# ruanjinchen/Point-Cloud-Flow-Matching

Hardware: AMD Instinct MI355X
Metric: train-step points/sec (B=8, N=20000, xyz+rgb) at 1/2/4/8 MI355X; Chamfer ms (higher is better)
Workload: dtype fp32 ContextNet (scatter/gather ops fp32; Conv3d + 1x1 convs as bf16x3 split-operand matrix-core products, fp32 accumulate, ~2^-16 per product vs the reference's default cuDNN TF32 2^-11) + bf16 autocast per-point MLP head (reference AMP config; its per-cloud B-row layers -- embeddings, FiLM affines

## Files before the change

### point-cloud-flow-matching_amd/csrc/rows.hpp

```cpp
#pragma once

#include <algorithm>

#include "bn_chan.hpp"
#include "pcfm_common.hpp"

namespace pcfm {


struct ProvIdx1 {
  static constexpr int TAPS = 1;
  const int* idx;
  int ni;
  int nrows;
  __device__ __forceinline__ void get(int b, int i, bool, int (&id)[1], float (&wt)[1]) const {
    const int v = idx[(size_t)b * ni + i];
    const bool ok = (unsigned)v < (unsigned)nrows;
    id[0] = ok ? v : 0;
    wt[0] = ok ? 1.0f : 0.0f;
  }
};

struct ProvDevox {
  static constexpr int TAPS = 8;
// ... 291 lines not shown
    int id[T];
    float w[T];
    prov.get(b, i, primary, id, w);
    const float4 a = tap_sum4<T>(lds4, id, w);
    const float r[4] = {a.x, a.y, a.z, a.w};
#pragma unroll
    for (int k = 0; k < 4; ++k) {
      float acc = r[k];
      if (epi.scale != nullptr) acc *= sc[k];
      if (ab != nullptr) acc += abn ? fa[k].z(ad[k]) : ad[k];
      ob[(size_t)k * NI + i] = acc;
    }
  }
}


struct RowPlan {
  int threads = 512;
  int cpb = 1;
  int groups = 1;
  int psplit = 1;
  bool use_lds = true;
  size_t lds_bytes = 0;
};

constexpr int kLdsFloatsSmall = 16 * 1024;
constexpr int kLdsFloatsBig = 32 * 1024;

constexpr long long kGatherTargetBlocks = 2 * kCUs;
constexpr int kGather1Ipt = 2;
// ... 17 lines not shown
  p.groups = groups(p.cpb);
  const long long blocks = (long long)p.groups * B;
  if (blocks < target) {
    const int want = ceil_div(target, blocks);
    const int cap = std::max(1, ceil_div(NI, p.threads));
    p.psplit = std::min(want, cap);
  }
  p.lds_bytes = p.use_lds ? (size_t)p.cpb * V * sizeof(float) : 0;
  return p;
}

template <class Prov>
inline bool prov_has_side_outputs(const Prov&) { return false; }
inline bool prov_has_side_outputs(const ProvDevox& p) { return p.inds_out != nullptr; }

template <class Prov>
inline int launch_gather(const float* rows, float* out, int B, int C, int V, int NI, Prov prov,
                         hipStream_t st, const char* what, GatherEpi epi = GatherEpi{},
                         BnParam bn = BnParam{}) {
  if (B == 0 || NI == 0) return PCFM_OK;
  if (V == 0 && C > 0 && epi.add == nullptr) {
    hipError_t e = hipMemsetAsync(out, 0, (size_t)B * C * NI * sizeof(float), st);
    if (e != hipSuccess) {
      set_error("%s: hipMemsetAsync: %s", what, hipGetErrorString(e));
      return (int)e;
    }
    if (!prov_has_side_outputs(prov)) return PCFM_OK;
  }
  RowPlan p = plan_gather(B, C, V, NI);
  dim3 grid(p.psplit, p.groups, B);
  if (p.use_lds && p.cpb == 4 && C % 4 == 0 && p.threads == 512) {
    int e = allow_big_lds((const void*)gather_rows4_kernel<Prov>);
    if (e) return e;
    hipLaunchKernelGGL((gather_rows4_kernel<Prov>), grid, dim3(512), p.lds_bytes, st, rows, out, C,
                       V, NI, prov, epi, bn);
  } else if (p.use_lds && p.cpb == 1 && p.threads == 1024) {
    int e = allow_big_lds((const void*)gather_rows1_kernel<Prov, kGather1Ipt>);
    if (e) return e;
    hipLaunchKernelGGL((gather_rows1_kernel<Prov, kGather1Ipt>), grid, dim3(1024), p.lds_bytes, st,
                       rows, out, C, V, NI, prov, epi, bn);
  } else if (p.use_lds) {
    int e = allow_big_lds((const void*)gather_rows_kernel<Prov, true>);
// ... 16 lines not shown
```

### point-cloud-flow-matching_amd/csrc/voxel.hip

```cpp
#include "rows.hpp"
#include "segsum.hpp"

namespace pcfm {
namespace {

__global__ void __launch_bounds__(256)
    vox_ind_kernel(const int* __restrict__ coords, int n, int r, int* __restrict__ ind) {
  const int b = blockIdx.y;
  const int i = blockIdx.x * blockDim.x + threadIdx.x;
  if (i >= n) return;
  const int* cb = coords + (size_t)b * 3 * n;
  ind[(size_t)b * n + i] = cb[i] * r * r + cb[i + n] * r + cb[i + 2 * n];
}

bool cube_fits(int r, int* s) {
  if (r < 1) return false;
  const long long c = (long long)r * r * r;
  if (c > (1LL << 30)) return false;
  *s = (int)c;
  return true;
}

__global__ void __launch_bounds__(256)
    rows_dot_kernel(const float* __restrict__ a, const float* __restrict__ b, int len, float scale,
// ... 334 lines not shown
extern "C" int pcfm_trilinear_devoxelize_bwd_planned(const float* grad_y, const void* plan, int b,
                                                     int c, int n, int r, float* grad_x, void* ws,
                                                     size_t ws_bytes, void* stream) {
  int s = 0;
  PCFM_CHECK_ARG(b >= 0 && c >= 0 && n >= 0, "trilinear_devoxelize_bwd_planned: negative size");
  PCFM_CHECK_ARG(cube_fits(r, &s), "trilinear_devoxelize_bwd_planned: bad resolution %d", r);
  PCFM_CHECK_ARG(plan != nullptr && ws_bytes >= seg_apply_bytes(b, c, n, s, 8),
                 "trilinear_devoxelize_bwd_planned: workspace too small");
  if (b == 0) return PCFM_OK;
  const int e = seg_apply(8, grad_y, seg_plan_carve(const_cast<void*>(plan), b, n, s, 8), false,
                          r, b, c, n, s, grad_x, seg_apply_carve(ws, b, c, n, s, 8),
                          (hipStream_t)stream);
  return e ? e : check_launch("trilinear_devoxelize_bwd_planned");
}

__device__ __forceinline__ float se_group_sum(float v) {
#pragma unroll
  for (int o = 8; o > 0; o >>= 1) v += __shfl_xor(v, o, 64);
  return v;
}

__global__ void __launch_bounds__(1024)
    se_mlp_fwd_kernel(const float* __restrict__ m, const float* __restrict__ w1,
                      const float* __restrict__ w2, int b, int c, int h, float* __restrict__ hid,
                      float* __restrict__ s) {
  extern __shared__ float sh[];
  float* ms = sh;
  float* w1s = ms + b * c;
  float* w2t = w1s + h * c;
  float* hs = w2t + h * c;
// ... 132 lines not shown
```

### point-cloud-flow-matching_amd/modules/functional/voxelization.py

```python
from torch.autograd import Function

from modules.functional import backend as _be



def _voxelize(feats, vox, r):
    if feats.is_cuda:
        from pcfm import ops, plans
        if plans.ENABLED:
            plan = plans.voxel_plan(vox, r)
            return ops.avg_voxelize_forward_planned(feats, plan), plan.ind, plan.cnt
    return _be._backend.avg_voxelize_forward(feats, vox, r)

__all__ = ["avg_voxelize", "avg_voxelize_tee"]


class AvgVoxelization(Function):

    @staticmethod
    def forward(ctx, features, coords, resolution):
        feats = features.contiguous()
        vox = coords.int().contiguous()
        b, c = feats.shape[0], feats.shape[1]
        r = int(resolution)
        grid, ind, cnt = _voxelize(feats, vox, r)
# ... 7 lines not shown
        flat = grad_output.contiguous().view(b, c, -1)
        return _be._backend.avg_voxelize_backward(flat, ind, cnt), None, None


avg_voxelize = AvgVoxelization.apply


class AvgVoxelizationTee(Function):

    @staticmethod
    def forward(ctx, features, coords, resolution):
        feats = features.contiguous()
        vox = coords.int().contiguous()
        b, c = feats.shape[0], feats.shape[1]
        r = int(resolution)
        grid, ind, cnt = _voxelize(feats, vox, r)
        ctx.save_for_backward(ind, cnt)
        return grid.view(b, c, r, r, r), features.view_as(features)

    @staticmethod
    def backward(ctx, grad_grid, grad_feat):
        from pcfm import ops
        ind, cnt = ctx.saved_tensors
        b, c = grad_grid.shape[0], grad_grid.shape[1]
        flat = grad_grid.contiguous().view(b, c, -1)
        if grad_feat is None:
            return _be._backend.avg_voxelize_backward(flat, ind, cnt), None, None
        return ops.avg_voxelize_backward_add(flat, ind, cnt, grad_feat), None, None


avg_voxelize_tee = AvgVoxelizationTee.apply
```

### point-cloud-flow-matching_amd/pcfm/_lib.py

```python
from __future__ import annotations

import ctypes
import os
import threading

_HERE = os.path.dirname(os.path.abspath(__file__))
LIB_PATH = os.path.join(os.path.dirname(_HERE), "csrc", "libpcfm_hip.so")
LIB_PATH = os.environ.get("PCFM_LIB", LIB_PATH)

_P = ctypes.c_void_p
_I = ctypes.c_int
_F = ctypes.c_float
_Z = ctypes.c_size_t
_L = ctypes.c_longlong
_D = ctypes.c_double
_DP = ctypes.POINTER(ctypes.c_double)

SIGNATURES = {
    "pcfm_abi_version": (_I, []),
    "pcfm_last_error": (ctypes.c_char_p, []),
    "pcfm_avg_voxelize_fwd_workspace_bytes": (_Z, [_I, _I, _I, _I]),
    "pcfm_avg_voxelize_fwd": (_I, [_P, _P, _I, _I, _I, _I, _P, _P, _P, _P, _Z, _P]),
    "pcfm_avg_voxelize_bwd": (_I, [_P, _P, _P, _I, _I, _I, _I, _P, _P]),
    "pcfm_trilinear_devoxelize_fwd": (_I, [_P, _P, _I, _I, _I, _I, _I, _P, _P, _P, _P]),
# ... 157 lines not shown
}

OCCUPANCY_ABI_VERSION = 1

EMD_ND_SIGNATURES = {
    "pcfm_emd_nd_abi_version": (_I, []),
    "pcfm_emd_nd_supported": (_I, [_I]),
    "pcfm_emd_nd_workspace_bytes": (_Z, [_I, _I, _I, _I]),
    "pcfm_emd_nd_approxmatch_cost_f32": (_I, [_P, _P, _I, _I, _I, _I, _P, _P, _P, _Z, _P]),
    "pcfm_emd_nd_matchcost_f32": (_I, [_P, _P, _P, _I, _I, _I, _I, _P, _P, _Z, _P]),
    "pcfm_emd_nd_matchcost_bwd_f32": (_I, [_P, _P, _P, _P, _I, _I, _I, _I, _P, _P, _P, _Z, _P]),
}

EMD_ND_ABI_VERSION = 1

_lock = threading.Lock()
_lib = None


class PcfmError(RuntimeError):
    """A pcfm_* entry point returned a non-zero status."""


def load() -> ctypes.CDLL:
    global _lib
    if _lib is not None:
        return _lib
    with _lock:
        if _lib is None:
            if not os.path.exists(LIB_PATH):
                raise RuntimeError(
                    f"pcfm: HIP library {LIB_PATH} is not built; run "
                    "`python -c 'import __graft_entry__ as g; g.build()'` "
                    "(HIP tensors have no fallback)")
            lib = ctypes.CDLL(LIB_PATH)
            for table in (SIGNATURES, ND_SIGNATURES, CROSS_SIGNATURES, FPS_SIGNATURES,
                          OCCUPANCY_SIGNATURES, EMD_ND_SIGNATURES):
                for name, (res, args) in table.items():
                    fn = getattr(lib, name)
                    fn.restype = res
                    fn.argtypes = args
            v = lib.pcfm_abi_version()
            if v != ABI_VERSION:
                raise RuntimeError(f"pcfm: ABI version {v} != expected {ABI_VERSION}; rebuild")
            v = lib.pcfm_chamfer_nd_abi_version()
            if v != ND_ABI_VERSION:
                raise RuntimeError(f"pcfm: chamfer_nd ABI version {v} != expected "
                                   f"{ND_ABI_VERSION}; rebuild")
            v = lib.pcfm_chamfer_cross_abi_version()
            if v != CROSS_ABI_VERSION:
                raise RuntimeError(f"pcfm: chamfer_cross ABI version {v} != expected "
                                   f"{CROSS_ABI_VERSION}; rebuild")
            v = lib.pcfm_fps_abi_version()
            if v != FPS_ABI_VERSION:
                raise RuntimeError(f"pcfm: fps ABI version {v} != expected "
                                   f"{FPS_ABI_VERSION}; rebuild")
            v = lib.pcfm_occupancy_abi_version()
            if v != OCCUPANCY_ABI_VERSION:
                raise RuntimeError(f"pcfm: occupancy ABI version {v} != expected "
                                   f"{OCCUPANCY_ABI_VERSION}; rebuild")
            v = lib.pcfm_emd_nd_abi_version()
            if v != EMD_ND_ABI_VERSION:
                raise RuntimeError(f"pcfm: emd_nd ABI version {v} != expected "
                                   f"{EMD_ND_ABI_VERSION}; rebuild")
            _lib = lib
    return _lib


def call(name: str, *args) -> None:
    lib = load()
    rc = getattr(lib, name)(*args)
    if rc != 0:
        msg = lib.pcfm_last_error().decode(errors="replace")
        raise PcfmError(f"{name} failed (status {rc}): {msg}")


def query(name: str, *args) -> int:
    return int(getattr(load(), name)(*args))
```

### point-cloud-flow-matching_amd/pcfm/ops.py

```python
from __future__ import annotations

import ctypes
import types

import torch

from . import _lib, cpu_ops


def _check_cuda(x: torch.Tensor, name: str) -> None:
    if not (isinstance(x, torch.Tensor) and x.is_cuda):
        raise RuntimeError(f"{name} must be a CUDA tensor")


def _check_contig(x: torch.Tensor, name: str) -> None:
    if not x.is_contiguous():
        raise RuntimeError(f"{name} must be a contiguous tensor")


def _check_float(x: torch.Tensor, name: str) -> None:
    if x.dtype != torch.float32:
        raise RuntimeError(f"{name} must be a float tensor")


# ... 88 lines not shown
    _check(coords, "coords", "i")
    b, c, n = features.shape
    r = int(resolution)
    s = r * r * r
    out = torch.empty((b, c, s), dtype=torch.float32, device=features.device)
    ind = torch.empty((b, n), dtype=torch.int32, device=features.device)
    cnt = torch.empty((b, s), dtype=torch.int32, device=features.device)
    ws = _workspace(_lib.query("pcfm_avg_voxelize_fwd_workspace_bytes", b, c, n, r), features)
    nbytes = 4 * b * (3 * n + c * n + n + s + c * s)
    with _timed("avg_voxelize_fwd", nbytes, features):
        _lib.call("pcfm_avg_voxelize_fwd", _ptr(features), _ptr(coords), b, c, n, r, _ptr(out),
                  _ptr(ind), _ptr(cnt), _ptr(ws), ws.numel(), _stream(features))
    return [out, ind, cnt]


def avg_voxelize_backward(grad_y: torch.Tensor, indices: torch.Tensor, cnt: torch.Tensor):
    if _host(grad_y, indices, cnt):
        _check_host(grad_y, "grad_y", "f")
        _check_host(indices, "indices", "i")
        _check_host(cnt, "cnt", "i")
        return cpu_ops.avg_voxelize_backward(grad_y, indices, cnt)
    _check(grad_y, "grad_y", "f")
    _check(indices, "indices", "i")
    _check(cnt, "cnt", "i")
    b, c, s = grad_y.shape
    n = indices.shape[1]
    grad_x = torch.empty((b, c, n), dtype=torch.float32, device=grad_y.device)
    nbytes = 4 * b * (c * s + n + s + c * n)
    with _timed("avg_voxelize_bwd", nbytes, grad_y):
        _lib.call("pcfm_avg_voxelize_bwd", _ptr(grad_y), _ptr(indices), _ptr(cnt), b, c, n, s,
                  _ptr(grad_x), _stream(grad_y))
    return grad_x


def avg_voxelize_backward_add(grad_y: torch.Tensor, indices: torch.Tensor, cnt: torch.Tensor,
                              add: torch.Tensor):
    _check(grad_y, "grad_y", "f")
    _check(indices, "indices", "i")
    _check(cnt, "cnt", "i")
    add = add.contiguous()
    _check(add, "add", "f")
    b, c, s = grad_y.shape
    n = indices.shape[1]
    if tuple(add.shape) != (b, c, n):
        raise ValueError("avg_voxelize_backward_add: add must be (B, C, N)")
    grad_x = torch.empty((b, c, n), dtype=torch.float32, device=grad_y.device)
    nbytes = 4 * b * (c * s + n + s + 2 * c * n)
    with _timed("avg_voxelize_bwd", nbytes, grad_y):
        _lib.call("pcfm_avg_voxelize_bwd_add", _ptr(grad_y), _ptr(indices), _ptr(cnt), _ptr(add),
                  b, c, n, s, _ptr(grad_x), _stream(grad_y))
    return grad_x


def trilinear_devoxelize_forward(r: int, is_training: bool, coords: torch.Tensor,
                                 features: torch.Tensor):
    if _host(coords, features):
        _check_host(features, "features", "f")
        _check_host(coords, "coords", "f")
        return cpu_ops.trilinear_devoxelize_forward(r, is_training, coords, features)
    _check(features, "features", "f")
    _check(coords, "coords", "f")
    b, c = features.shape[0], features.shape[1]
    n = coords.shape[2]
    r = int(r)
    dev = features.device
    outs = torch.empty((b, c, n), dtype=torch.float32, device=dev)
    if is_training:
        inds = torch.empty((b, 8, n), dtype=torch.int32, device=dev)
        wgts = torch.empty((b, 8, n), dtype=torch.float32, device=dev)
        pi, pw = _ptr(inds), _ptr(wgts)
    else:
        inds = torch.zeros((1,), dtype=torch.int32, device=dev)
        wgts = torch.zeros((1,), dtype=torch.float32, device=dev)
        pi, pw = None, None
    nbytes = 4 * b * (3 * n + c * r ** 3 + c * n + (16 * n if is_training else 0))
    with _timed("trilinear_devoxelize_fwd", nbytes, features):
        _lib.call("pcfm_trilinear_devoxelize_fwd", _ptr(coords), _ptr(features), b, c, n, r,
                  1 if is_training else 0, _ptr(outs), pi, pw, _stream(features))
    if devox_verify.enabled:
        devox_verify(coords, features, None, None, outs, inds if is_training else None,
                     wgts if is_training else None, r)
    return [outs, inds, wgts]


def trilinear_devoxelize_scale_add(r: int, is_training: bool, coords: torch.Tensor,
                                   features: torch.Tensor, scale, add):
    _check(features, "features", "f")
    _check(coords, "coords", "f")
    b, c = features.shape[0], features.shape[1]
    n = coords.shape[2]
    r = int(r)
    dev = features.device
    if scale is not None:
# ... 6 lines not shown
        _check(add, "add", "f")
        if tuple(add.shape) != (b, c, n):
            raise ValueError("trilinear_devoxelize_scale_add: add must be (B, C, N)")
    outs = torch.empty((b, c, n), dtype=torch.float32, device=dev)
    if is_training:
        inds = torch.empty((b, 8, n), dtype=torch.int32, device=dev)
        wgts = torch.empty((b, 8, n), dtype=torch.float32, device=dev)
        pi, pw = _ptr(inds), _ptr(wgts)
    else:
        inds = torch.zeros((1,), dtype=torch.int32, device=dev)
        wgts = torch.zeros((1,), dtype=torch.float32, device=dev)
        pi, pw = None, None
    nbytes = 4 * b * (3 * n + c * r ** 3 + c * n * (2 if add is not None else 1)
                      + (16 * n if is_training else 0))
    with _timed("trilinear_devoxelize_fwd", nbytes, features):
        _lib.call("pcfm_trilinear_devoxelize_scale_add_fwd", _ptr(coords), _ptr(features),
                  _ptr(scale) if scale is not None else None,
                  _ptr(add) if add is not None else None, b, c, n, r, 1 if is_training else 0,
                  _ptr(outs), pi, pw, _stream(features))
    if devox_verify.enabled:
        devox_verify(coords, features, scale, add, outs, inds if is_training else None,
                     wgts if is_training else None, r)
    return [outs, inds, wgts]


class _DevoxVerify:

    def __init__(self):
        import os
        self.enabled = os.environ.get("PCFM_DEVOX_VERIFY") == "1"
        self.rec = None
        self.calls = 0

    def __call__(self, coords, features, scale, add, outs, inds, wgts, r):
# ... 28 lines not shown
            return {"calls": self.calls, "mismatches": 0, "bad_weight_sums": 0, "records": []}
        h = self.rec.cpu().tolist()
        recs = []
        for k in range(min(h[0], 16)):
            e = h[2 + 8 * k: 10 + 8 * k]
            recs.append({"kind": ("out", "ind", "wgt")[e[0]], "b": e[1], "c": e[2], "i": e[3],
                         "got_bits": e[4], "want_bits": e[5], "lane": e[6], "wave_of_i": e[7]})
        return {"calls": self.calls, "mismatches": h[0], "bad_weight_sums": h[1], "records": recs}


devox_verify = _DevoxVerify()


class SegPlan:

    __slots__ = ("buf", "b", "n", "r", "taps", "ind", "cnt")

    def __init__(self, buf, b, n, r, taps, ind=None, cnt=None):
        self.buf, self.b, self.n, self.r, self.taps = buf, b, n, r, taps
        self.ind, self.cnt = ind, cnt


def avg_voxelize_plan(coords: torch.Tensor, resolution: int) -> SegPlan:
    _check(coords, "coords", "i")
    b, n = coords.shape[0], coords.shape[2]
    r = int(resolution)
    dev = coords.device
    ind = torch.empty((b, n), dtype=torch.int32, device=dev)
    cnt = torch.empty((b, r ** 3), dtype=torch.int32, device=dev)
    buf = _workspace(_lib.query("pcfm_seg_plan_bytes", b, n, r, 1), coords)
    with _timed("avg_voxelize_plan", 4 * b * (3 * n + 3 * n + 2 * r ** 3), coords):
        _lib.call("pcfm_avg_voxelize_plan", _ptr(coords), b, n, r, _ptr(ind), _ptr(cnt), _ptr(buf),
                  buf.numel(), _stream(coords))
    return SegPlan(buf, b, n, r, 1, ind, cnt)

# ... 1075 lines not shown
        pi, pw = None, None
    nbytes = 4 * b * (3 * n + c * r ** 3 + c * n * (2 if add is not None else 1)
                      + (16 * n if is_training else 0))
    abn = [None, None, None, None]
    aslope = 0.0
    if add_bn is not None:
        if add is None:
            raise ValueError("trilinear_devoxelize_bn_scale_add: add_bn without add")
        for t in add_bn[:4]:
            _check(t, "add_bn", "f")
            if t.numel() != c:
                raise ValueError("trilinear_devoxelize_bn_scale_add: add_bn entries must have C values")
        abn = [_ptr(t) for t in add_bn[:4]]
        aslope = float(add_bn[4])
    with _timed("trilinear_devoxelize_fwd", nbytes, x):
        _lib.call("pcfm_trilinear_devoxelize_bn_scale_add_fwd", _ptr(coords), _ptr(x), _ptr(mean),
                  _ptr(invstd), _ptr(weight), _ptr(bias), float(slope),
                  _ptr(scale) if scale is not None else None,
                  _ptr(add) if add is not None else None, *abn, aslope, b, c, n, r,
                  1 if is_training else 0, _ptr(outs), pi, pw, _stream(x))
    if devox_verify.enabled:
        devox_verify.bn(coords, x, (mean, invstd, weight, bias, slope), scale, add, add_bn, outs,
                        inds if is_training else None, wgts if is_training else None, r)
    return [outs, inds, wgts]


def bn_forward_stats(x: torch.Tensor, eps: float, momentum: float, running_mean, running_var,
                     num_batches_tracked=None, parts=None):
    _check(x, "input", "f")
    b, c = x.shape[0], x.shape[1]
    s = x.numel() // max(1, b * c)
    stats = torch.empty((2, c), dtype=torch.float32, device=x.device)
    if parts is not None:
        _check(parts, "parts", "f")
        ws = _workspace(1, x)
# ... 190 lines not shown
```

### point-cloud-flow-matching_amd/pcfm/plans.py

```python
from __future__ import annotations

import os
import weakref
from typing import NamedTuple, Optional

import torch

ENABLED = os.environ.get("PCFM_SHARE_PLANS", "1") != "0"
OCCUPANCY = os.environ.get("PCFM_CONV_OCC", "1") != "0"
VOXEL_LISTS = os.environ.get("PCFM_CONV_VLIST", "1") != "0"


class Occupancy(NamedTuple):
    masks: torch.Tensor
    lists: Optional[torch.Tensor]
    cnt: torch.Tensor


class IdentityCache:

    def __init__(self):
        self._d = {}

    def get(self, t: torch.Tensor, tag):
# ... 68 lines not shown
        return None
    occ = Occupancy(masks, ops.conv3d_vlists(cnt, r) if VOXEL_LISTS else None, cnt)
    _cache.put(vox_coords, tag, (occ,))
    return occ


def devox_corners(norm_coords: torch.Tensor, r: int):
    return _cache.get(norm_coords, ("corners", int(r))) if _on(norm_coords) else None


def put_devox_corners(norm_coords: torch.Tensor, r: int, inds, wgts) -> None:
    if _on(norm_coords):
        _cache.put(norm_coords, ("corners", int(r)), (inds, wgts))


def devox_bwd_plan(norm_coords: torch.Tensor, inds: torch.Tensor, wgts: torch.Tensor, r: int):
    from pcfm import ops
    tag = ("devox_bwd", int(r))
    hit = _cache.get(norm_coords, tag) if _on(norm_coords) else None
    if hit is not None:
        return hit
    plan = ops.trilinear_devoxelize_backward_plan(inds, wgts, r)
    return _cache.put(norm_coords, tag, plan) if _on(norm_coords) else plan
```

Baseline: 5.702 million.

## Gather devoxelize and voxelize-backward rows through compacted occupied-voxel LDS staging

Adds a compact-plan path for trilinear devoxelize forward and avg-voxelize backward when V lies between 16K and 32K floats. It builds a per-cloud list of occupied voxels and per-point slot indices, then stages only the occupied voxels for 4 or 2 channels at once in LDS. This lets each block process more channels per pass than whole-row staging allows. The cost is extra plan-building kernels, which are cached per coords tensor, and more code complexity.

```diff
diff --git a/include/pcfm_gather_compact.h b/include/pcfm_gather_compact.h
--- /dev/null
+++ b/include/pcfm_gather_compact.h
@@ -0,0 +1,41 @@
+#ifndef PCFM_GATHER_COMPACT_H
+#define PCFM_GATHER_COMPACT_H
+
+#include <stddef.h>
+
+#ifdef __cplusplus
+extern "C" {
+#endif
+
+#define PCFM_GATHER_COMPACT_ABI_VERSION 1
+
+int pcfm_gather_compact_abi_version(void);
+
+int pcfm_gather_compact_supported(int c, int r);
+
+int pcfm_gather_compact_slots(int width);
+
+size_t pcfm_gather_compact_plan_bytes(int b, int n, int r, int taps);
+
+int pcfm_trilinear_devoxelize_compact_plan(const float* coords, int b, int n, int r, void* plan,
+                                           size_t plan_bytes, void* stream);
+
+int pcfm_avg_voxelize_compact_plan(const int* ind, const int* cnt, int b, int n, int r, void* plan,
+                                   size_t plan_bytes, void* stream);
+
+int pcfm_trilinear_devoxelize_compact_fwd(
+    const float* coords, const float* x, const float* bn_mean, const float* bn_invstd,
+    const float* gamma, const float* beta, float slope, const float* scale, const float* add,
+    const float* add_mean, const float* add_invstd, const float* add_gamma,
+    const float* add_beta, float add_slope, const void* plan, size_t plan_bytes, int b, int c,
+    int n, int r, int training, float* out, int* inds, float* wgts, void* stream);
+
+int pcfm_avg_voxelize_compact_bwd(const float* grad_y, const int* ind, const int* cnt,
+                                  const float* add, const void* plan, size_t plan_bytes, int b,
+                                  int c, int n, int r, float* grad_x, void* stream);
+
+#ifdef __cplusplus
+}
+#endif
+
+#endif
diff --git a/point-cloud-flow-matching_amd/csrc/rows.hpp b/point-cloud-flow-matching_amd/csrc/rows.hpp
--- a/point-cloud-flow-matching_amd/csrc/rows.hpp
+++ b/point-cloud-flow-matching_amd/csrc/rows.hpp
@@ -1,6 +1,8 @@
 #pragma once
 
 #include <algorithm>
+#include <cstdlib>
+#include <type_traits>
 
 #include "bn_chan.hpp"
 #include "pcfm_common.hpp"
@@ -329,6 +331,187 @@
   }
 }
 
+struct CompactPlan {
+  const int* count = nullptr;
+  const unsigned short* list = nullptr;
+  const void* items = nullptr;
+};
+
+constexpr int kCompactLdsBytes = kLdsBytesMax - 1024;
+constexpr int kCompactSlots4 = kCompactLdsBytes / 16;
+constexpr int kCompactSlots2 = kCompactLdsBytes / 8;
+constexpr int kCompactMaxV = 32 * 1024;
+static_assert(kCompactLdsBytes >= 4 * kCompactMaxV, "the whole-row fallback must fit");
+
+struct CompactLayout {
+  size_t count, list, items, bits, rank, total;
+  int words;
+};
+inline size_t compact_rnd(size_t x) { return (x + 255) & ~(size_t)255; }
+inline CompactLayout compact_layout(int b, int n, int V, int taps) {
+  CompactLayout L;
+  L.words = ceil_div(V, 32);
+  L.count = 0;
+  L.list = compact_rnd(4 * (size_t)b);
+  L.items = L.list + compact_rnd(2 * (size_t)b * V);
+  L.bits = L.items + compact_rnd((size_t)b * n * (taps == 8 ? 16 : 8));
+  L.rank = L.bits + compact_rnd(4 * (size_t)b * L.words);
+  L.total = L.rank + compact_rnd(4 * (size_t)b * L.words);
+  return L;
+}
+inline CompactPlan compact_carve(const void* plan, int b, int n, int V, int taps) {
+  const CompactLayout L = compact_layout(b, n, V, taps);
+  const char* p = static_cast<const char*>(plan);
+  CompactPlan cp;
+  cp.count = reinterpret_cast<const int*>(p + L.count);
+  cp.list = reinterpret_cast<const unsigned short*>(p + L.list);
+  cp.items = p + L.items;
+  return cp;
+}
+
+__device__ __forceinline__ void compact_get(const ProvDevox& prov, const CompactPlan& cp, int b,
+                                            int i, bool primary, int cnt, int (&slot)[8],
+                                            float (&w)[8]) {
+  const uint4 q = reinterpret_cast<const uint4*>(cp.items)[(size_t)b * prov.n + i];
+  int id[8];
+  prov.get(b, i, primary, id, w);
+  const unsigned h[4] = {q.x, q.y, q.z, q.w};
+#pragma unroll
+  for (int k = 0; k < 4; ++k) {
+    slot[2 * k] = min((int)(h[k] & 0xffffu), cnt - 1);
+    slot[2 * k + 1] = min((int)(h[k] >> 16), cnt - 1);
+  }
+}
+__device__ __forceinline__ void compact_get(const ProvVoxBwd& prov, const CompactPlan& cp, int b,
+                                            int i, bool, int cnt, int (&slot)[1], float (&w)[1]) {
+  const uint2 q = reinterpret_cast<const uint2*>(cp.items)[(size_t)b * prov.n + i];
+  slot[0] = (int)min(q.x, (unsigned)(cnt - 1));
+  w[0] = __uint_as_float(q.y);
+}
+
+template <int T>
+__device__ __forceinline__ float2 tap_sum2(const float2* __restrict__ s, const int (&id)[T],
+                                           const float (&w)[T]) {
+  if constexpr (T == 1) {
+    const float2 v = s[id[0]];
+    return make_float2(v.x * w[0], v.y * w[0]);
+  } else {
+    const float2 v1 = s[id[1]], v0 = s[id[0]];
+    float2 a = make_float2(w[1] * v1.x, w[1] * v1.y);
+    a.x = __builtin_fmaf(w[0], v0.x, a.x);
+    a.y = __builtin_fmaf(w[0], v0.y, a.y);
+#pragma unroll
+    for (int k = 2; k < T; ++k) {
+      const float2 v = s[id[k]];
+      a.x = __builtin_fmaf(w[k], v.x, a.x);
+      a.y = __builtin_fmaf(w[k], v.y, a.y);
+    }
+    return a;
+  }
+}
+
+template <class Prov, int W>
+__device__ __forceinline__ void compact_pass(const float* __restrict__ rows,
+                                             float* __restrict__ out, float* lds, int b, int cb,
+                                             int C, int V, int NI, int cnt,
+                                             const unsigned short* __restrict__ list,
+                                             const Prov& prov, const GatherEpi& epi,
+                                             const BnParam& bn, const CompactPlan& cp,
+                                             bool primary) {
+  constexpr int T = Prov::TAPS;
+  const float* __restrict__ rb = rows + ((size_t)b * C + cb) * V;
+  BnChan f[W];
+#pragma unroll
+  for (int k = 0; k < W; ++k) f[k] = bn.at_or_identity(cb + k);
+  const bool rbn = bn.mean != nullptr;
+  if constexpr (W == 1) {
+    for (int e = threadIdx.x; e < V; e += blockDim.x) lds[e] = rbn ? f[0].z(rb[e]) : rb[e];
+  } else {
+    for (int s0 = threadIdx.x; s0 < cnt; s0 += 4 * blockDim.x) {
+      float v[4][W];
+#pragma unroll
+      for (int u = 0; u < 4; ++u) {
+        const int s = min(s0 + u * (int)blockDim.x, cnt - 1);
+        const int vox = min((int)list[s], V - 1);
+#pragma unroll
+        for (int k = 0; k < W; ++k) v[u][k] = rb[(size_t)k * V + vox];
+      }
+#pragma unroll
+      for (int u = 0; u < 4; ++u) {
+        const int s = s0 + u * (int)blockDim.x;
+        if (s < cnt) {
+#pragma unroll
+          for (int k = 0; k < W; ++k) lds[(size_t)s * W + k] = rbn ? f[k].z(v[u][k]) : v[u][k];
+        }
+      }
+    }
+  }
+  __syncthreads();
+  float* __restrict__ ob = out + ((size_t)b * C + cb) * NI;
+  const float* __restrict__ ab = epi.add != nullptr ? epi.add + ((size_t)b * C + cb) * NI : nullptr;
+  float sc[W];
+  BnChan fa[W];
+#pragma unroll
+  for (int k = 0; k < W; ++k) {
+    sc[k] = epi.scale != nullptr ? epi.scale[(size_t)b * C + cb + k] : 1.0f;
+    fa[k] = add_bn_at(epi, cb + k);
+  }
+  const bool abn = epi.add_bn.mean != nullptr;
+  for (int i = blockIdx.x * blockDim.x + threadIdx.x; i < NI; i += gridDim.x * blockDim.x) {
+    float ad[W];
+#pragma unroll
+    for (int k = 0; k < W; ++k) ad[k] = ab != nullptr ? nt_ld(ab + (size_t)k * NI + i) : 0.0f;
+    int id[T];
+    float w[T];
+    float r[W];
+    if constexpr (W == 1) {
+      prov.get(b, i, primary, id, w);
+      r[0] = tap_sum<T>(lds, id, w);
+    } else {
+      compact_get(prov, cp, b, i, primary, cnt, id, w);
+      if constexpr (W == 4) {
+        const float4 a = tap_sum4<T>(reinterpret_cast<const float4*>(lds), id, w);
+        r[0] = a.x, r[1] = a.y, r[2] = a.z, r[3] = a.w;
+      } else {
+        const float2 a = tap_sum2<T>(reinterpret_cast<const float2*>(lds), id, w);
+        r[0] = a.x, r[1] = a.y;
+      }
+    }
+#pragma unroll
+    for (int k = 0; k < W; ++k) {
+      float acc = r[k];
+      if (epi.scale != nullptr) acc *= sc[k];
+      if (ab != nullptr) acc += abn ? fa[k].z(ad[k]) : ad[k];
+      ob[(size_t)k * NI + i] = acc;
+    }
+  }
+}
+
+template <class Prov>
+__global__ void __launch_bounds__(1024)
+    gather_compact4_kernel(const float* __restrict__ rows, float* __restrict__ out, int C, int V,
+                           int NI, Prov prov, GatherEpi epi, BnParam bn, CompactPlan cp) {
+  extern __shared__ __attribute__((aligned(16))) float lds[];
+  const int b = blockIdx.z;
+  const int c0 = blockIdx.y * 4;
+  const int cnt = max(1, min(cp.count[b], V));
+  const unsigned short* __restrict__ list = cp.list + (size_t)b * V;
+  const bool primary = blockIdx.y == 0;
+  if (cnt <= kCompactSlots4) {
+    compact_pass<Prov, 4>(rows, out, lds, b, c0, C, V, NI, cnt, list, prov, epi, bn, cp, primary);
+  } else if (cnt <= kCompactSlots2) {
+    compact_pass<Prov, 2>(rows, out, lds, b, c0, C, V, NI, cnt, list, prov, epi, bn, cp, primary);
+    __syncthreads();
+    compact_pass<Prov, 2>(rows, out, lds, b, c0 + 2, C, V, NI, cnt, list, prov, epi, bn, cp, false);
+  } else {
+    for (int k = 0; k < 4; ++k) {
+      if (k > 0) __syncthreads();
+      compact_pass<Prov, 1>(rows, out, lds, b, c0 + k, C, V, NI, cnt, list, prov, epi, bn, cp,
+                            primary && k == 0);
+    }
+  }
+}
+
 
 struct RowPlan {
   int threads = 512;
@@ -376,10 +559,26 @@
 inline bool prov_has_side_outputs(const Prov&) { return false; }
 inline bool prov_has_side_outputs(const ProvDevox& p) { return p.inds_out != nullptr; }
 
+inline bool gather_compact_enabled() {
+  static const bool on = [] {
+    const char* e = std::getenv("PCFM_GATHER_COMPACT");
+    return !(e != nullptr && e[0] == '0');
+  }();
+  return on;
+}
+
+inline bool gather_compact_class(int C, int V) {
+  return C > 0 && C % 4 == 0 && V > kLdsFloatsSmall && V <= kLdsFloatsBig;
+}
+
+#ifndef PCFM_COMPACT_TARGET
+#define PCFM_COMPACT_TARGET kCUs
+#endif
+
 template <class Prov>
 inline int launch_gather(const float* rows, float* out, int B, int C, int V, int NI, Prov prov,
                          hipStream_t st, const char* what, GatherEpi epi = GatherEpi{},
-                         BnParam bn = BnParam{}) {
+                         BnParam bn = BnParam{}, CompactPlan cp = CompactPlan{}) {
   if (B == 0 || NI == 0) return PCFM_OK;
   if (V == 0 && C > 0 && epi.add == nullptr) {
     hipError_t e = hipMemsetAsync(out, 0, (size_t)B * C * NI * sizeof(float), st);
@@ -388,6 +587,18 @@
       return (int)e;
     }
     if (!prov_has_side_outputs(prov)) return PCFM_OK;
+  }
+  if constexpr (std::is_same_v<Prov, ProvDevox> || std::is_same_v<Prov, ProvVoxBwd>) {
+    if (cp.count != nullptr && gather_compact_enabled() && gather_compact_class(C, V)) {
+      const long long blocks = (long long)(C / 4) * B;
+      const int want = std::max(1, ceil_div(PCFM_COMPACT_TARGET, blocks));
+      const int psplit = std::min(want, std::max(1, ceil_div(NI, 1024)));
+      int e = allow_big_lds((const void*)gather_compact4_kernel<Prov>);
+      if (e) return e;
+      hipLaunchKernelGGL((gather_compact4_kernel<Prov>), dim3(psplit, C / 4, B), dim3(1024),
+                         kCompactLdsBytes, st, rows, out, C, V, NI, prov, epi, bn, cp);
+      return check_launch(what);
+    }
   }
   RowPlan p = plan_gather(B, C, V, NI);
   dim3 grid(p.psplit, p.groups, B);
diff --git a/point-cloud-flow-matching_amd/csrc/voxel.hip b/point-cloud-flow-matching_amd/csrc/voxel.hip
--- a/point-cloud-flow-matching_amd/csrc/voxel.hip
+++ b/point-cloud-flow-matching_amd/csrc/voxel.hip
@@ -1,3 +1,4 @@
+#include "../../include/pcfm_gather_compact.h"
 #include "rows.hpp"
 #include "segsum.hpp"
 
@@ -372,6 +373,260 @@
   return e ? e : check_launch("trilinear_devoxelize_bwd_planned");
 }
 
+namespace pcfm {
+namespace {
+
+constexpr int kCompactWords = kCompactMaxV / 32;
+
+template <bool FROM_CNT>
+__global__ void __launch_bounds__(1024)
+    compact_list_kernel(ProvDevox prov, const int* __restrict__ cnt, int n, int V, int words,
+                        int* __restrict__ count, unsigned short* __restrict__ list,
+                        unsigned* __restrict__ bits, int* __restrict__ rank) {
+  __shared__ unsigned sbits[kCompactWords];
+  __shared__ int wsum[16];
+  const int b = blockIdx.x, t = threadIdx.x;
+  const int lane = t & 63, wave = t >> 6;
+  sbits[t] = 0u;
+  __syncthreads();
+  if constexpr (FROM_CNT) {
+    const int* __restrict__ cb = cnt + (size_t)b * V;
+    for (int base0 = wave * 64; base0 < words * 32; base0 += 4 * 1024) {
+      int cv[4];
+#pragma unroll
+      for (int u = 0; u < 4; ++u) {
+        const int v = base0 + u * 1024 + lane;
+        cv[u] = v < V ? cb[v] : 0;
+      }
+#pragma unroll
+      for (int u = 0; u < 4; ++u) {
+        const int base = base0 + u * 1024;
+        const unsigned long long m = __ballot(cv[u] > 0);
+        if (lane == 0 && base < words * 32) {
+          sbits[base >> 5] = (unsigned)m;
+          if ((base >> 5) + 1 < words) sbits[(base >> 5) + 1] = (unsigned)(m >> 32);
+        }
+      }
+    }
+  } else {
+    for (int i0 = t; i0 < n; i0 += 2 * 1024) {
+      int id[2][8];
+      float w[8];
+      const int i1 = i0 + 1024 < n ? i0 + 1024 : i0;
+      prov.get(b, i0, false, id[0], w);
+      prov.get(b, i1, false, id[1], w);
+#pragma unroll
+      for (int u = 0; u < 2; ++u) {
+#pragma unroll
+        for (int k = 0; k < 8; ++k) {
+          const unsigned v = min((unsigned)id[u][k], (unsigned)(V - 1));
+          atomicOr(&sbits[v >> 5], 1u << (v & 31));
+        }
+      }
+    }
+  }
+  __syncthreads();
+  unsigned my = t < words ? sbits[t] : 0u;
+  if (t == 0) my |= 1u;
+  const int pc = __popc(my);
+  int incl = pc;
+#pragma unroll
+  for (int o = 1; o < 64; o <<= 1) {
+    const int up = __shfl_up(incl, o, 64);
+    if (lane >= o) incl += up;
+  }
+  if (lane == 63) wsum[wave] = incl;
+  __syncthreads();
+  int before = 0, total = 0;
+#pragma unroll
+  for (int k = 0; k < 16; ++k) {
+    const int s = wsum[k];
+    before += k < wave ? s : 0;
+    total += s;
+  }
+  const int excl = before + incl - pc;
+  if (t < words) {
+    bits[(size_t)b * words + t] = my;
+    rank[(size_t)b * words + t] = excl;
+    unsigned short* __restrict__ lb = list + (size_t)b * V;
+    int s = excl;
+    for (unsigned m = my; m != 0u; m &= m - 1u) lb[s++] = (unsigned short)(32 * t + __ffs(m) - 1);
+  }
+  if (t == 0) count[b] = total;
+}
+
+__device__ __forceinline__ unsigned compact_slot(const unsigned* __restrict__ bits,
+                                                 const int* __restrict__ rank, int words,
+                                                 int id) {
+  const unsigned v = min((unsigned)id, 32u * (unsigned)words - 1u);
+  return (unsigned)rank[v >> 5] + (unsigned)__popc(bits[v >> 5] & ((1u << (v & 31)) - 1u));
+}
+
+__global__ void __launch_bounds__(256)
+    compact_items8_kernel(ProvDevox prov, int words, const unsigned* __restrict__ bits,
+                          const int* __restrict__ rank, uint4* __restrict__ items) {
+  const int b = blockIdx.y;
+  const int i = blockIdx.x * blockDim.x + threadIdx.x;
+  if (i >= prov.n) return;
+  int id[8];
+  float w[8];
+  prov.get(b, i, false, id, w);
+  unsigned s[8];
+#pragma unroll
+  for (int k = 0; k < 8; ++k)
+    s[k] = compact_slot(bits + (size_t)b * words, rank + (size_t)b * words, words, id[k]);
+  items[(size_t)b * prov.n + i] =
+      make_uint4(s[0] | (s[1] << 16), s[2] | (s[3] << 16), s[4] | (s[5] << 16), s[6] | (s[7] << 16));
+}
+
+__global__ void __launch_bounds__(256)
+    compact_items1_kernel(ProvVoxBwd prov, int words, const unsigned* __restrict__ bits,
+                          const int* __restrict__ rank, uint2* __restrict__ items) {
+  const int b = blockIdx.y;
+  const int i = blockIdx.x * blockDim.x + threadIdx.x;
+  if (i >= prov.n) return;
+  int id[1];
+  float w[1];
+  prov.get(b, i, false, id, w);
+  items[(size_t)b * prov.n + i] = make_uint2(
+      compact_slot(bits + (size_t)b * words, rank + (size_t)b * words, words, id[0]),
+      __float_as_uint(w[0]));
+}
+
+bool compact_sizes_ok(int b, int n, int r, int* s) {
+  return b >= 0 && n >= 0 && cube_fits(r, s) && *s <= kCompactMaxV &&
+         (long long)b * n < (1LL << 27);
+}
+
+struct CompactBuild {
+  int* count;
+  unsigned short* list;
+  void* items;
+  unsigned* bits;
+  int* rank;
+  int words;
+};
+CompactBuild compact_build_carve(void* plan, int b, int n, int V, int taps) {
+  const CompactLayout L = compact_layout(b, n, V, taps);
+  char* p = static_cast<char*>(plan);
+  return CompactBuild{reinterpret_cast<int*>(p + L.count),
+                      reinterpret_cast<unsigned short*>(p + L.list), p + L.items,
+                      reinterpret_cast<unsigned*>(p + L.bits), reinterpret_cast<int*>(p + L.rank),
+                      L.words};
+}
+
+}
+}
+
+extern "C" int pcfm_gather_compact_abi_version(void) { return PCFM_GATHER_COMPACT_ABI_VERSION; }
+
+extern "C" int pcfm_gather_compact_supported(int c, int r) {
+  int s = 0;
+  return cube_fits(r, &s) && gather_compact_class(c, s) && gather_compact_enabled() ? 1 : 0;
+}
+
+extern "C" int pcfm_gather_compact_slots(int width) {
+  return width == 4 ? kCompactSlots4 : width == 2 ? kCompactSlots2 : 0;
+}
+
+extern "C" size_t pcfm_gather_compact_plan_bytes(int b, int n, int r, int taps) {
+  int s = 0;
+  if (!compact_sizes_ok(b, n, r, &s) || !plan_taps_ok(taps)) return 0;
+  return compact_layout(b, n, s, taps).total;
+}
+
+extern "C" int pcfm_trilinear_devoxelize_compact_plan(const float* coords, int b, int n, int r,
+                                                      void* plan, size_t plan_bytes,
+                                                      void* stream) {
+  int s = 0;
+  PCFM_CHECK_ARG(compact_sizes_ok(b, n, r, &s),
+                 "trilinear_devoxelize_compact_plan: bad size b=%d n=%d r=%d", b, n, r);
+  PCFM_CHECK_ARG(plan != nullptr && ((uintptr_t)plan & 15) == 0 &&
+                     plan_bytes >= compact_layout(b, n, s, 8).total,
+                 "trilinear_devoxelize_compact_plan: plan buffer too small or misaligned");
+  if (b == 0) return PCFM_OK;
+  hipStream_t st = (hipStream_t)stream;
+  const CompactBuild p = compact_build_carve(plan, b, n, s, 8);
+  const ProvDevox prov{coords, n, r, r * r, s, nullptr, nullptr};
+  hipLaunchKernelGGL(compact_list_kernel<false>, dim3(b), dim3(1024), 0, st, prov, nullptr, n, s,
+                     p.words, p.count, p.list, p.bits, p.rank);
+  if (n > 0)
+    hipLaunchKernelGGL(compact_items8_kernel, dim3(ceil_div(n, 256), b), dim3(256), 0, st, prov,
+                       p.words, p.bits, p.rank, static_cast<uint4*>(p.items));
+  return check_launch("trilinear_devoxelize_compact_plan");
+}
+
+extern "C" int pcfm_avg_voxelize_compact_plan(const int* ind, const int* cnt, int b, int n, int r,
+                                              void* plan, size_t plan_bytes, void* stream) {
+  int s = 0;
+  PCFM_CHECK_ARG(compact_sizes_ok(b, n, r, &s),
+                 "avg_voxelize_compact_plan: bad size b=%d n=%d r=%d", b, n, r);
+  PCFM_CHECK_ARG(plan != nullptr && ((uintptr_t)plan & 15) == 0 &&
+                     plan_bytes >= compact_layout(b, n, s, 1).total,
+                 "avg_voxelize_compact_plan: plan buffer too small or misaligned");
+  if (b == 0) return PCFM_OK;
+  hipStream_t st = (hipStream_t)stream;
+  const CompactBuild p = compact_build_carve(plan, b, n, s, 1);
+  hipLaunchKernelGGL(compact_list_kernel<true>, dim3(b), dim3(1024), 0, st, ProvDevox{}, cnt, n, s,
+                     p.words, p.count, p.list, p.bits, p.rank);
+  if (n > 0)
+    hipLaunchKernelGGL(compact_items1_kernel, dim3(ceil_div(n, 256), b), dim3(256), 0, st,
+                       ProvVoxBwd{ind, cnt, n, s}, p.words, p.bits, p.rank,
+                       static_cast<uint2*>(p.items));
+  return check_launch("avg_voxelize_compact_plan");
+}
+
+extern "C" int pcfm_trilinear_devoxelize_compact_fwd(
+    const float* coords, const float* x, const float* bn_mean, const float* bn_invstd,
+    const float* gamma, const float* beta, float slope, const float* scale, const float* add,
+    const float* add_mean, const float* add_invstd, const float* add_gamma,
+    const float* add_beta, float add_slope, const void* plan, size_t plan_bytes, int b, int c,
+    int n, int r, int training, float* out, int* inds, float* wgts, void* stream) {
+  int s = 0;
+  PCFM_CHECK_ARG(c >= 0 && compact_sizes_ok(b, n, r, &s),
+                 "trilinear_devoxelize_compact_fwd: bad size b=%d c=%d n=%d r=%d", b, c, n, r);
+  PCFM_CHECK_ARG(bn_mean == nullptr ||
+                     (bn_invstd != nullptr && gamma != nullptr && beta != nullptr),
+                 "trilinear_devoxelize_compact_fwd: incomplete BatchNorm operands");
+  PCFM_CHECK_ARG(!training || (long long)b * n == 0 || (inds != nullptr && wgts != nullptr),
+                 "trilinear_devoxelize_compact_fwd: training needs inds/wgts buffers");
+  PCFM_CHECK_ARG(add_mean == nullptr ||
+                     (add != nullptr && add_invstd != nullptr && add_gamma != nullptr &&
+                      add_beta != nullptr),
+                 "trilinear_devoxelize_compact_fwd: incomplete BatchNorm operands of add");
+  PCFM_CHECK_ARG(plan != nullptr && ((uintptr_t)plan & 15) == 0 &&
+                     plan_bytes >= compact_layout(b, n, s, 8).total,
+                 "trilinear_devoxelize_compact_fwd: plan buffer too small or misaligned");
+  ProvDevox prov{coords, n, r, r * r, s, training ? inds : nullptr, training ? wgts : nullptr};
+  GatherEpi epi;
+  epi.scale = scale;
+  epi.add = add;
+  epi.add_bn = BnParam{add_mean, add_invstd, add_gamma, add_beta, add_slope};
+  const BnParam bn = bn_mean != nullptr ? BnParam{bn_mean, bn_invstd, gamma, beta, slope}
+                                        : BnParam{};
+  return launch_gather(x, out, b, c, s, n, prov, (hipStream_t)stream,
+                       "trilinear_devoxelize_compact_fwd", epi, bn,
+                       compact_carve(plan, b, n, s, 8));
+}
+
+extern "C" int pcfm_avg_voxelize_compact_bwd(const float* grad_y, const int* ind, const int* cnt,
+                                             const float* add, const void* plan,
+                                             size_t plan_bytes, int b, int c, int n, int r,
+                                             float* grad_x, void* stream) {
+  int s = 0;
+  PCFM_CHECK_ARG(c >= 0 && compact_sizes_ok(b, n, r, &s),
+                 "avg_voxelize_compact_bwd: bad size b=%d c=%d n=%d r=%d", b, c, n, r);
+  PCFM_CHECK_ARG(plan != nullptr && ((uintptr_t)plan & 15) == 0 &&
+                     plan_bytes >= compact_layout(b, n, s, 1).total,
+                 "avg_voxelize_compact_bwd: plan buffer too small or misaligned");
+  if (c == 0) return PCFM_OK;
+  GatherEpi epi;
+  epi.add = add;
+  return launch_gather(grad_y, grad_x, b, c, s, n, ProvVoxBwd{ind, cnt, n, s},
+                       (hipStream_t)stream, "avg_voxelize_compact_bwd", epi, BnParam{},
+                       compact_carve(plan, b, n, s, 1));
+}
+
 __device__ __forceinline__ float se_group_sum(float v) {
 #pragma unroll
   for (int o = 8; o > 0; o >>= 1) v += __shfl_xor(v, o, 64);
diff --git a/point-cloud-flow-matching_amd/modules/functional/voxelization.py b/point-cloud-flow-matching_amd/modules/functional/voxelization.py
--- a/point-cloud-flow-matching_amd/modules/functional/voxelization.py
+++ b/point-cloud-flow-matching_amd/modules/functional/voxelization.py
@@ -4,11 +4,13 @@
 
 
 
-def _voxelize(feats, vox, r):
+def _voxelize(feats, vox, r, ctx=None):
     if feats.is_cuda:
         from pcfm import ops, plans
         if plans.ENABLED:
             plan = plans.voxel_plan(vox, r)
+            if ctx is not None:
+                ctx.seg_plan = plan
             return ops.avg_voxelize_forward_planned(feats, plan), plan.ind, plan.cnt
     return _be._backend.avg_voxelize_forward(feats, vox, r)
 
@@ -46,7 +48,8 @@
         vox = coords.int().contiguous()
         b, c = feats.shape[0], feats.shape[1]
         r = int(resolution)
-        grid, ind, cnt = _voxelize(feats, vox, r)
+        ctx.seg_plan = None
+        grid, ind, cnt = _voxelize(feats, vox, r, ctx)
         ctx.save_for_backward(ind, cnt)
         return grid.view(b, c, r, r, r), features.view_as(features)
 
@@ -58,7 +61,7 @@
         flat = grad_grid.contiguous().view(b, c, -1)
         if grad_feat is None:
             return _be._backend.avg_voxelize_backward(flat, ind, cnt), None, None
-        return ops.avg_voxelize_backward_add(flat, ind, cnt, grad_feat), None, None
+        return ops.avg_voxelize_backward_add(flat, ind, cnt, grad_feat, ctx.seg_plan), None, None
 
 
 avg_voxelize_tee = AvgVoxelizationTee.apply
diff --git a/point-cloud-flow-matching_amd/pcfm/_lib.py b/point-cloud-flow-matching_amd/pcfm/_lib.py
--- a/point-cloud-flow-matching_amd/pcfm/_lib.py
+++ b/point-cloud-flow-matching_amd/pcfm/_lib.py
@@ -195,6 +195,22 @@
 
 EMD_ND_ABI_VERSION = 1
 
+GATHER_COMPACT_SIGNATURES = {
+    "pcfm_gather_compact_abi_version": (_I, []),
+    "pcfm_gather_compact_supported": (_I, [_I, _I]),
+    "pcfm_gather_compact_slots": (_I, [_I]),
+    "pcfm_gather_compact_plan_bytes": (_Z, [_I, _I, _I, _I]),
+    "pcfm_trilinear_devoxelize_compact_plan": (_I, [_P, _I, _I, _I, _P, _Z, _P]),
+    "pcfm_avg_voxelize_compact_plan": (_I, [_P, _P, _I, _I, _I, _P, _Z, _P]),
+    "pcfm_trilinear_devoxelize_compact_fwd": (_I, [_P, _P, _P, _P, _P, _P, _F, _P, _P, _P, _P,
+                                                   _P, _P, _F, _P, _Z, _I, _I, _I, _I, _I, _P,
+                                                   _P, _P, _P]),
+    "pcfm_avg_voxelize_compact_bwd": (_I, [_P, _P, _P, _P, _P, _Z, _I, _I, _I, _I, _P, _P]),
+}
+
+GATHER_COMPACT_ABI_VERSION = 1
+HAS_GATHER_COMPACT = True
+
 _lock = threading.Lock()
 _lib = None
 
@@ -215,8 +231,14 @@
                     "`python -c 'import __graft_entry__ as g; g.build()'` "
                     "(HIP tensors have no fallback)")
             lib = ctypes.CDLL(LIB_PATH)
-            for table in (SIGNATURES, ND_SIGNATURES, CROSS_SIGNATURES, FPS_SIGNATURES,
-                          OCCUPANCY_SIGNATURES, EMD_ND_SIGNATURES):
+            tables = [SIGNATURES, ND_SIGNATURES, CROSS_SIGNATURES, FPS_SIGNATURES,
+                      OCCUPANCY_SIGNATURES, EMD_ND_SIGNATURES]
+            global HAS_GATHER_COMPACT
+            HAS_GATHER_COMPACT = ("PCFM_LIB" not in os.environ
+                                  or hasattr(lib, "pcfm_gather_compact_abi_version"))
+            if HAS_GATHER_COMPACT:
+                tables.append(GATHER_COMPACT_SIGNATURES)
+            for table in tables:
                 for name, (res, args) in table.items():
                     fn = getattr(lib, name)
                     fn.restype = res
@@ -244,6 +266,10 @@
             if v != EMD_ND_ABI_VERSION:
                 raise RuntimeError(f"pcfm: emd_nd ABI version {v} != expected "
                                    f"{EMD_ND_ABI_VERSION}; rebuild")
+            v = lib.pcfm_gather_compact_abi_version() if HAS_GATHER_COMPACT else 1
+            if v != GATHER_COMPACT_ABI_VERSION:
+                raise RuntimeError(f"pcfm: gather_compact ABI version {v} != expected "
+                                   f"{GATHER_COMPACT_ABI_VERSION}; rebuild")
             _lib = lib
     return _lib
 
diff --git a/point-cloud-flow-matching_amd/pcfm/ops.py b/point-cloud-flow-matching_amd/pcfm/ops.py
--- a/point-cloud-flow-matching_amd/pcfm/ops.py
+++ b/point-cloud-flow-matching_amd/pcfm/ops.py
@@ -126,6 +126,61 @@
     return [out, ind, cnt]
 
 
+def gather_compact_supported(c: int, r: int) -> bool:
+    _lib.load()
+    return (_lib.HAS_GATHER_COMPACT
+            and _lib.query("pcfm_gather_compact_supported", int(c), int(r)) == 1)
+
+
+def trilinear_devoxelize_compact_plan(coords: torch.Tensor, r: int) -> torch.Tensor:
+    _check(coords, "coords", "f")
+    b, n = coords.shape[0], coords.shape[2]
+    buf = _workspace(_lib.query("pcfm_gather_compact_plan_bytes", b, n, int(r), 8), coords)
+    _lib.call("pcfm_trilinear_devoxelize_compact_plan", _ptr(coords), b, n, int(r), _ptr(buf),
+              buf.numel(), _stream(coords))
+    return buf
+
+
+def avg_voxelize_compact_plan(indices: torch.Tensor, cnt: torch.Tensor, r: int) -> torch.Tensor:
+    _check(indices, "indices", "i")
+    _check(cnt, "cnt", "i")
+    b, n = indices.shape
+    buf = _workspace(_lib.query("pcfm_gather_compact_plan_bytes", b, n, int(r), 1), indices)
+    _lib.call("pcfm_avg_voxelize_compact_plan", _ptr(indices), _ptr(cnt), b, n, int(r), _ptr(buf),
+              buf.numel(), _stream(indices))
+    return buf
+
+
+def _cube_root(s: int) -> int:
+    r = round(s ** (1.0 / 3.0))
+    return r if r ** 3 == s else 0
+
+
+def _vox_bwd(grad_y, indices, cnt, add, plan):
+    b, c, s = grad_y.shape
+    n = indices.shape[1]
+    grad_x = torch.empty((b, c, n), dtype=torch.float32, device=grad_y.device)
+    nbytes = 4 * b * (c * s + n + s + (2 if add is not None else 1) * c * n)
+    r = _cube_root(s)
+    with _timed("avg_voxelize_bwd", nbytes, grad_y):
+        if r and b * n and gather_compact_supported(c, r):
+            cp = plan.compact if plan is not None else None
+            if cp is None:
+                cp = avg_voxelize_compact_plan(indices, cnt, r)
+                if plan is not None:
+                    plan.compact = cp
+            _lib.call("pcfm_avg_voxelize_compact_bwd", _ptr(grad_y), _ptr(indices), _ptr(cnt),
+                      _ptr(add) if add is not None else None, _ptr(cp), cp.numel(), b, c, n, r,
+                      _ptr(grad_x), _stream(grad_y))
+        elif add is not None:
+            _lib.call("pcfm_avg_voxelize_bwd_add", _ptr(grad_y), _ptr(indices), _ptr(cnt),
+                      _ptr(add), b, c, n, s, _ptr(grad_x), _stream(grad_y))
+        else:
+            _lib.call("pcfm_avg_voxelize_bwd", _ptr(grad_y), _ptr(indices), _ptr(cnt), b, c, n, s,
+                      _ptr(grad_x), _stream(grad_y))
+    return grad_x
+
+
 def avg_voxelize_backward(grad_y: torch.Tensor, indices: torch.Tensor, cnt: torch.Tensor):
     if _host(grad_y, indices, cnt):
         _check_host(grad_y, "grad_y", "f")
@@ -135,18 +190,11 @@
     _check(grad_y, "grad_y", "f")
     _check(indices, "indices", "i")
     _check(cnt, "cnt", "i")
-    b, c, s = grad_y.shape
-    n = indices.shape[1]
-    grad_x = torch.empty((b, c, n), dtype=torch.float32, device=grad_y.device)
-    nbytes = 4 * b * (c * s + n + s + c * n)
-    with _timed("avg_voxelize_bwd", nbytes, grad_y):
-        _lib.call("pcfm_avg_voxelize_bwd", _ptr(grad_y), _ptr(indices), _ptr(cnt), b, c, n, s,
-                  _ptr(grad_x), _stream(grad_y))
-    return grad_x
+    return _vox_bwd(grad_y, indices, cnt, None, None)
 
 
 def avg_voxelize_backward_add(grad_y: torch.Tensor, indices: torch.Tensor, cnt: torch.Tensor,
-                              add: torch.Tensor):
+                              add: torch.Tensor, plan=None):
     _check(grad_y, "grad_y", "f")
     _check(indices, "indices", "i")
     _check(cnt, "cnt", "i")
@@ -156,12 +204,25 @@
     n = indices.shape[1]
     if tuple(add.shape) != (b, c, n):
         raise ValueError("avg_voxelize_backward_add: add must be (B, C, N)")
-    grad_x = torch.empty((b, c, n), dtype=torch.float32, device=grad_y.device)
-    nbytes = 4 * b * (c * s + n + s + 2 * c * n)
-    with _timed("avg_voxelize_bwd", nbytes, grad_y):
-        _lib.call("pcfm_avg_voxelize_bwd_add", _ptr(grad_y), _ptr(indices), _ptr(cnt), _ptr(add),
-                  b, c, n, s, _ptr(grad_x), _stream(grad_y))
-    return grad_x
+    return _vox_bwd(grad_y, indices, cnt, add, plan)
+
+
+def _devox_compact(coords, b, c, n, r):
+    if not (b * n and gather_compact_supported(c, r)):
+        return None
+    from . import plans
+    return plans.devox_compact(coords, r)
+
+
+def _devox_compact_fwd(cp, coords, x, bn, slope, scale, add, abn, aslope, b, c, n, r, training,
+                       outs, pi, pw):
+    _lib.call("pcfm_trilinear_devoxelize_compact_fwd", _ptr(coords), _ptr(x), *bn, float(slope),
+              _ptr(scale) if scale is not None else None,
+              _ptr(add) if add is not None else None, *abn, float(aslope), _ptr(cp), cp.numel(),
+              b, c, n, r, 1 if training else 0, _ptr(outs), pi, pw, _stream(x))
+
+
+_NO_BN = (None, None, None, None)
 
 
 def trilinear_devoxelize_forward(r: int, is_training: bool, coords: torch.Tensor,
@@ -187,8 +248,13 @@
         pi, pw = None, None
     nbytes = 4 * b * (3 * n + c * r ** 3 + c * n + (16 * n if is_training else 0))
     with _timed("trilinear_devoxelize_fwd", nbytes, features):
-        _lib.call("pcfm_trilinear_devoxelize_fwd", _ptr(coords), _ptr(features), b, c, n, r,
-                  1 if is_training else 0, _ptr(outs), pi, pw, _stream(features))
+        cp = _devox_compact(coords, b, c, n, r)
+        if cp is not None:
+            _devox_compact_fwd(cp, coords, features, _NO_BN, 0.0, None, None, _NO_BN, 0.0, b, c,
+                               n, r, is_training, outs, pi, pw)
+        else:
+            _lib.call("pcfm_trilinear_devoxelize_fwd", _ptr(coords), _ptr(features), b, c, n, r,
+                      1 if is_training else 0, _ptr(outs), pi, pw, _stream(features))
     if devox_verify.enabled:
         devox_verify(coords, features, None, None, outs, inds if is_training else None,
                      wgts if is_training else None, r)
@@ -225,10 +291,15 @@
     nbytes = 4 * b * (3 * n + c * r ** 3 + c * n * (2 if add is not None else 1)
                       + (16 * n if is_training else 0))
     with _timed("trilinear_devoxelize_fwd", nbytes, features):
-        _lib.call("pcfm_trilinear_devoxelize_scale_add_fwd", _ptr(coords), _ptr(features),
-                  _ptr(scale) if scale is not None else None,
-                  _ptr(add) if add is not None else None, b, c, n, r, 1 if is_training else 0,
-                  _ptr(outs), pi, pw, _stream(features))
+        cp = _devox_compact(coords, b, c, n, r)
+        if cp is not None:
+            _devox_compact_fwd(cp, coords, features, _NO_BN, 0.0, scale, add, _NO_BN, 0.0, b, c,
+                               n, r, is_training, outs, pi, pw)
+        else:
+            _lib.call("pcfm_trilinear_devoxelize_scale_add_fwd", _ptr(coords), _ptr(features),
+                      _ptr(scale) if scale is not None else None,
+                      _ptr(add) if add is not None else None, b, c, n, r,
+                      1 if is_training else 0, _ptr(outs), pi, pw, _stream(features))
     if devox_verify.enabled:
         devox_verify(coords, features, scale, add, outs, inds if is_training else None,
                      wgts if is_training else None, r)
@@ -287,11 +358,12 @@
 
 class SegPlan:
 
-    __slots__ = ("buf", "b", "n", "r", "taps", "ind", "cnt")
+    __slots__ = ("buf", "b", "n", "r", "taps", "ind", "cnt", "compact")
 
     def __init__(self, buf, b, n, r, taps, ind=None, cnt=None):
         self.buf, self.b, self.n, self.r, self.taps = buf, b, n, r, taps
         self.ind, self.cnt = ind, cnt
+        self.compact = None
 
 
 def avg_voxelize_plan(coords: torch.Tensor, resolution: int) -> SegPlan:
@@ -1397,11 +1469,17 @@
         abn = [_ptr(t) for t in add_bn[:4]]
         aslope = float(add_bn[4])
     with _timed("trilinear_devoxelize_fwd", nbytes, x):
-        _lib.call("pcfm_trilinear_devoxelize_bn_scale_add_fwd", _ptr(coords), _ptr(x), _ptr(mean),
-                  _ptr(invstd), _ptr(weight), _ptr(bias), float(slope),
-                  _ptr(scale) if scale is not None else None,
-                  _ptr(add) if add is not None else None, *abn, aslope, b, c, n, r,
-                  1 if is_training else 0, _ptr(outs), pi, pw, _stream(x))
+        cp = _devox_compact(coords, b, c, n, r)
+        if cp is not None:
+            _devox_compact_fwd(cp, coords, x, (_ptr(mean), _ptr(invstd), _ptr(weight), _ptr(bias)),
+                               slope, scale, add, abn, aslope, b, c, n, r, is_training, outs, pi,
+                               pw)
+        else:
+            _lib.call("pcfm_trilinear_devoxelize_bn_scale_add_fwd", _ptr(coords), _ptr(x),
+                      _ptr(mean), _ptr(invstd), _ptr(weight), _ptr(bias), float(slope),
+                      _ptr(scale) if scale is not None else None,
+                      _ptr(add) if add is not None else None, *abn, aslope, b, c, n, r,
+                      1 if is_training else 0, _ptr(outs), pi, pw, _stream(x))
     if devox_verify.enabled:
         devox_verify.bn(coords, x, (mean, invstd, weight, bias, slope), scale, add, add_bn, outs,
                         inds if is_training else None, wgts if is_training else None, r)
diff --git a/point-cloud-flow-matching_amd/pcfm/plans.py b/point-cloud-flow-matching_amd/pcfm/plans.py
--- a/point-cloud-flow-matching_amd/pcfm/plans.py
+++ b/point-cloud-flow-matching_amd/pcfm/plans.py
@@ -106,6 +106,16 @@
         _cache.put(norm_coords, ("corners", int(r)), (inds, wgts))
 
 
+def devox_compact(norm_coords: torch.Tensor, r: int):
+    from pcfm import ops
+    tag = ("devox_compact", int(r))
+    hit = _cache.get(norm_coords, tag) if _on(norm_coords) else None
+    if hit is not None:
+        return hit
+    plan = ops.trilinear_devoxelize_compact_plan(norm_coords, r)
+    return _cache.put(norm_coords, tag, plan) if _on(norm_coords) else plan
+
+
 def devox_bwd_plan(norm_coords: torch.Tensor, inds: torch.Tensor, wgts: torch.Tensor, r: int):
     from pcfm import ops
     tag = ("devox_bwd", int(r))
```

After: 5.734 million (median of 6 runs). About the same (+0.6%).
